# thomasahle/tinyknn

Hardware: AMD Instinct MI355X
Metric: queries/sec at Recall10@10 on GloVe-100 angular (synthetic stand-in), IVF+4-bit PQ, build_probes=1 (higher is better)
Workload: dtype int8 (saturating PQ sums) + f32 (tables, rescoring); 1 GPU; glove-100-angular stand-in: 300 Gaussian clusters sigma 0.7, N=1183514 d=100 IVF n_clusters=1087 build_probes=1 FastPQ dpb=2 M=52; k=10, n_probes=10, parallelism=replica x1 (queries sharded), batches_in_flight=2

## Files before the change

tinyknn_amd/csrc/heap.hip:

```cpp
#include <stdlib.h>

#include <type_traits>

#include "kernels.h"

typedef __attribute__((address_space(3))) volatile uint32_t lds_vu32;
typedef __attribute__((address_space(3))) volatile int32_t lds_vi32;
typedef __attribute__((address_space(3))) volatile int64_t lds_vi64;
#define LDS_PTR(T, p) ((T *)(__attribute__((address_space(3))) unsigned char *)(p))

template <bool SIGNED>
__device__ __forceinline__ bool byte_lt(uint32_t d, uint32_t bound8)
{
    if (SIGNED) return (int)(int8_t)d < (int)(int8_t)bound8;
    return d < bound8;
}

template <bool SIGNED>
__device__ __forceinline__ bool any_lt16(const uint4 v, uint32_t bound8)
{
    const uint32_t w[4] = {v.x, v.y, v.z, v.w};
    bool any = false;
#pragma unroll
    for (int i = 0; i < 4; i++)
// ... 266 lines not shown
#pragma unroll
        for (int i = 0; i < 4; i++) {
            const uint4 dd = dd4[i];
            uint64_t mask = __builtin_amdgcn_ballot_w64(byte_lt<SIGNED>(mn4[i], bound));
            while (mask) {
                const int j = __builtin_ctzll(mask);
                mask &= mask - 1;
                const uint32_t d0 = __builtin_amdgcn_readlane(dd.x, j);
                const uint32_t d1 = __builtin_amdgcn_readlane(dd.y, j);
                const uint32_t d2 = __builtin_amdgcn_readlane(dd.z, j);
                const uint32_t d3 = __builtin_amdgcn_readlane(dd.w, j);
                const int64_t pos0 = 16 * (int64_t)__builtin_amdgcn_readlane(bm4[i], j);
                const uint32_t wr = lane < 4 ? d0 : lane < 8 ? d1 : lane < 12 ? d2 : d3;
                const uint32_t myb = (wr >> (8 * (lane & 3))) & 0xffu;
                uint32_t bits = (uint32_t)__builtin_amdgcn_ballot_w64(lane < 16 && byte_lt<SIGNED>(myb, bound));
                while (bits) {
                    const int r = __builtin_ctz(bits);
                    bits &= bits - 1;
                    const int64_t pos = pos0 + r;
                    if (pos < n) {
                        const uint32_t w = r < 4 ? d0 : r < 8 ? d1 : r < 12 ? d2 : d3;
                        const uint32_t by = (w >> (8 * (r & 3))) & 0xffu;
                        reg_heap_insert(H, K, pos, SIGNED ? (int32_t)(int8_t)by : (int32_t)by);
                    }
                }
                bound = (uint32_t)__builtin_amdgcn_readlane(H.v, 0) & 0xffu;
                if (mask) mask &= __builtin_amdgcn_ballot_w64(byte_lt<SIGNED>(mn4[i], bound));
            }
        }
    }
}

template <bool SIGNED>
__global__ __launch_bounds__(1024) void flat_top_one_kernel(const uint4 *__restrict__ dist,
                                                            const uint8_t *__restrict__ mins, int chunks, int h,
                                                            int64_t n, int R, uint4 *__restrict__ cdist,
                                                            int *__restrict__ cblock, int64_t *__restrict__ out_idx,
                                                            int32_t *__restrict__ out_val)
{
#ifdef TK_FLAT_CLOCK
    int64_t *dbg = (int64_t *)(out_idx + 1024);
    int n_ins = 0;
#define CLK(i) if (tid == 0) { dbg[2 * (i)] = __builtin_readcyclecounter(); dbg[2 * (i) + 1] = __builtin_amdgcn_s_memrealtime(); }
#else
#define CLK(i)
#endif
    __shared__ uint32_t s_bound;
    __shared__ int s_wave[16], s_total;
    const int tid = threadIdx.x, lane = tid & 63, wave = tid >> 6;
    RegHeap H = {SIGNED ? 127 : 255, 0xffffffffu, 0xffffffffu};
    uint32_t bound = SIGNED ? 127u : 255u;
    const RegHeapLane K = reg_heap_lane(lane, R);
    const int rest = chunks - h;
    const int per = ((rest + 1023) / 1024 + 15) & ~15;
    const int b_lo = h + tid * per;
    uint4 pm[4];
#pragma unroll
    for (int g = 0; g < 4; g++) {
        const int b0 = b_lo + 16 * g;
        pm[g] = make_uint4(0, 0, 0, 0);
        if (16 * g < per && b0 < chunks) pm[g] = *(const uint4 *)(mins + b0);
    }
    CLK(0)
    if (wave == 0) {
        reg_heap_span<SIGNED>(H, K, bound, dist, mins, h, nullptr, n, lane);
        if (lane == 0) s_bound = bound;
    }
    CLK(1)
    __syncthreads();
    const uint32_t hb = s_bound;
    uint8_t *cmin = (uint8_t *)(cblock + chunks);
    uint64_t keep = 0;
#pragma unroll
    for (int g = 0; g < 4; g++) {
        const uint32_t w[4] = {pm[g].x, pm[g].y, pm[g].z, pm[g].w};
#pragma unroll
        for (int k = 0; k < 16; k++)
            keep |= (uint64_t)byte_lt<SIGNED>((w[k >> 2] >> (8 * (k & 3))) & 0xffu, hb) << (16 * g + k);
    }
    {
        int valid = per < 64 ? per : 64;
        if (b_lo + valid > chunks) valid = chunks - b_lo;
        keep = valid <= 0 ? 0 : valid >= 64 ? keep : keep & ((1ull << valid) - 1ull);
    }
    int cnt = __builtin_popcountll(keep);
    for (int g = 64; g < per; g += 16) {
        const int b0 = b_lo + g;
        if (b0 >= chunks) break;
        const uint4 m16 = *(const uint4 *)(mins + b0);
        const uint32_t w[4] = {m16.x, m16.y, m16.z, m16.w};
#pragma unroll
        for (int k = 0; k < 16; k++)
            cnt += (b0 + k < chunks) && byte_lt<SIGNED>((w[k >> 2] >> (8 * (k & 3))) & 0xffu, hb);
    }
    int inc = cnt;
#pragma unroll
    for (int o = 1; o < 64; o <<= 1) {
        const int up = __shfl_up(inc, o, 64);
        if (lane >= o) inc += up;
    }
    if (lane == 63) s_wave[wave] = inc;
    __syncthreads();
    int at = inc - cnt;
    for (int w = 0; w < wave; w++) at += s_wave[w];
    if (tid == 1023) s_total = at + cnt;
    while (keep) {
        const int b = b_lo + __builtin_ctzll(keep);
        keep &= keep - 1;
        cdist[at] = dist[b];
        cblock[at] = b;
        cmin[at] = mins[b];
        at++;
    }
    for (int g = 64; g < per; g += 16) {
        const int b0 = b_lo + g;
        if (b0 >= chunks) break;
        const uint4 m16 = *(const uint4 *)(mins + b0);
        const uint32_t w[4] = {m16.x, m16.y, m16.z, m16.w};
#pragma unroll
        for (int k = 0; k < 16; k++)
            if ((b0 + k < chunks) && byte_lt<SIGNED>((w[k >> 2] >> (8 * (k & 3))) & 0xffu, hb)) {
                cdist[at] = dist[b0 + k];
                cblock[at] = b0 + k;
                cmin[at] = (uint8_t)((w[k >> 2] >> (8 * (k & 3))) & 0xffu);
                at++;
            }
    }
    __threadfence();
    __syncthreads();
    if (wave != 0) return;
    CLK(2)
    reg_heap_span<SIGNED>(H, K, bound, cdist, cmin, s_total, cblock, n, lane);
    CLK(3)
#ifdef TK_FLAT_CLOCK
    if (tid == 0) dbg[8] = s_total;
#endif
    if (lane < R) {
        out_idx[lane] = (int64_t)(((uint64_t)H.hi << 32) | H.lo);
        out_val[lane] = H.v;
    }
}

void tk_launch_flat_top_one(const uint4 *dist, const uint8_t *mins, int chunks, int h, int64_t n, int R, int signd,
                            uint4 *cdist, int *cblock, int64_t *out_idx, int32_t *out_val, hipStream_t s)
{
    if (signd)
        hipLaunchKernelGGL(flat_top_one_kernel<true>, dim3(1), dim3(1024), 0, s, dist, mins, chunks, h, n, R, cdist,
                           cblock, out_idx, out_val);
    else
        hipLaunchKernelGGL(flat_top_one_kernel<false>, dim3(1), dim3(1024), 0, s, dist, mins, chunks, h, n, R, cdist,
                           cblock, out_idx, out_val);
}

#ifndef TK_LANES_SEG
#define TK_LANES_SEG 8
#endif
template <bool SIGNED>
__device__ __forceinline__ int entry_val(uint32_t e)
{
    return SIGNED ? ((int32_t)e >> 24) : (int)(e >> 24);
}

template <bool SIGNED>
__device__ __forceinline__ uint32_t mask_lt16(const uint4 v, uint32_t bound8)
{
    const uint32_t w[4] = {v.x, v.y, v.z, v.w};
    uint32_t m = 0;
#pragma unroll
    for (int i = 0; i < 4; i++)
#pragma unroll
        for (int b = 0; b < 4; b++)
            m |= (uint32_t)byte_lt<SIGNED>((w[i] >> (8 * b)) & 0xffu, bound8) << (4 * i + b);
    return m;
}

template <bool SIGNED>
__device__ __forceinline__ uint32_t bound_bytes(uint32_t bound8)
{
    const uint32_t b = SIGNED ? (bound8 ^ 0x80u) : bound8;
    return __builtin_amdgcn_perm(b, b, 0u);
}

template <bool SIGNED>
__device__ __forceinline__ uint32_t lt4(uint32_t x, uint32_t bb, uint32_t bl)
{
    const uint32_t H = 0x80808080u;
    const uint32_t xu = SIGNED ? (x ^ H) : x;
    const uint32_t t = (xu | H) - bl;
    return ((~xu & bb) | (~(xu ^ bb) & ~t)) & H;
}

template <bool SIGNED>
__device__ __forceinline__ uint32_t mask_lt16_swar(const uint4 v, uint32_t bb)
{
    const uint32_t bl = bb & 0x7f7f7f7fu;
    uint32_t lo = __builtin_amdgcn_udot4(lt4<SIGNED>(v.x, bb, bl), 0x08040201u, 0u, false);
    lo = __builtin_amdgcn_udot4(lt4<SIGNED>(v.y, bb, bl), 0x80402010u, lo, false);
    uint32_t hi = __builtin_amdgcn_udot4(lt4<SIGNED>(v.z, bb, bl), 0x08040201u, 0u, false);
    hi = __builtin_amdgcn_udot4(lt4<SIGNED>(v.w, bb, bl), 0x80402010u, hi, false);
    return (lo >> 7) | (hi << 1);
}

template <bool SIGNED>
__global__ void pad_fix_kernel(uint4 *__restrict__ dist, int64_t cap, int64_t nq,
                               const int *__restrict__ slot_prefix, const int *__restrict__ slot_n,
                               int S, int slots_uniform, uint8_t *__restrict__ mins, int64_t cap_min,
                               int *__restrict__ flag_list)
{
    const int64_t i = (int64_t)blockIdx.x * blockDim.x + threadIdx.x;
    if (i == 0 && flag_list) flag_list[0] = 0;
    if (i >= nq * S) return;
    const int64_t q = i / S;
    const int sl = (int)(i - q * S);
    const int64_t qs = slots_uniform ? 0 : q;
    const int f0 = slot_prefix[qs * (S + 1) + sl], f1 = slot_prefix[qs * (S + 1) + sl + 1];
    int n = slot_n[qs * S + sl];
    n = n < 0 ? 0 : n;
    const uint32_t fill = SIGNED ? 0x7f7f7f7fu : 0xffffffffu;
    for (int c = n >> 4; c < f1 - f0; c++) {
        const int keep = n - 16 * c;
        uint4 v = dist[q * cap + f0 + c];
        uint32_t w[4] = {v.x, v.y, v.z, v.w};
        int m = SIGNED ? 127 : 255;
#pragma unroll
        for (int j = 0; j < 4; j++) {
            int km = keep - 4 * j;
            km = km < 0 ? 0 : (km > 4 ? 4 : km);
            const uint32_t kmask = km >= 4 ? 0xffffffffu : ((1u << (8 * km)) - 1u);
            w[j] = (w[j] & kmask) | (fill & ~kmask);
#pragma unroll
            for (int t = 0; t < 4; t++) {
                const uint32_t b = (w[j] >> (8 * t)) & 0xffu;
                const int x = SIGNED ? (int)(int8_t)b : (int)b;
                m = x < m ? x : m;
            }
        }
        dist[q * cap + f0 + c] = make_uint4(w[0], w[1], w[2], w[3]);
        mins[q * cap_min + f0 + c] = (uint8_t)m;
    }
}

template <bool SIGNED, bool DEDUPE, int LW, bool LAZY = false, bool TWIN = false>
__global__ __launch_bounds__(256) void heap_replay_lanes_kernel(
    const uint4 *__restrict__ dist, int64_t cap, int64_t nq, const int *__restrict__ slot_prefix,
    const int *__restrict__ slot_n, const int64_t *__restrict__ slot_label_off, int S,
    const int64_t *__restrict__ labels, int64_t *__restrict__ heap_idx,
    int32_t *__restrict__ heap_val, int R, int slots_uniform,
    unsigned char *__restrict__ skip, int nbuf, const uint8_t *__restrict__ mins,
    int64_t cap_min, const int32_t *__restrict__ labels32, unsigned long long *__restrict__ dbg,
    int prio, int wave_lds, const int *__restrict__ plain0_arr, const int *__restrict__ qlim, const TkTwins tw,
    int *__restrict__ flag_list)
{
    static_assert(!(TWIN && DEDUPE), "one form of the duplicate test");
    if ((prio & 0xff) >= 3) __builtin_amdgcn_s_setprio(3);
    else if ((prio & 0xff) == 2) __builtin_amdgcn_s_setprio(2);
    else if ((prio & 0xff) == 1) __builtin_amdgcn_s_setprio(1);
    extern __shared__ __attribute__((aligned(16))) unsigned char smem_wg[];
    unsigned char *smem = smem_wg + (size_t)(threadIdx.x >> 6) * wave_lds;
    uint32_t *H = (uint32_t *)smem;
    const int R4 = (R + 3) >> 2;
    constexpr size_t CB = (size_t)LW * 4;
    uint32_t *LAB = (uint32_t *)(smem + (size_t)(R + 2) * CB);
    uint4 *TB = (uint4 *)(smem + (size_t)(R + 2) * CB + (size_t)R4 * CB * 4);
    uint4 *ST = (uint4 *)(smem + (size_t)(R + 2) * CB +
                          (DEDUPE ? (size_t)R4 * CB * 4 + (size_t)64 * CB * 4 : 0));
    int *SE = (int *)(ST + (DEDUPE ? 16 : LAZY ? 0 : TWIN ? 16 : TK_LANES_SEG) * LW);
    int *SB = SE + (size_t)S * LW;
    uint4 *PL = (uint4 *)(SB + (size_t)S * LW);
    const int S4 = (S + 3) >> 2;
    uint32_t *BM = (uint32_t *)(PL + (size_t)S4 * LW);
    const int BMW = TWIN ? tw.bm_words : 0;
#define TK_LAB(slot) LAB[(((slot) >> 2) * LW + lane) * 4 + ((slot) & 3)]
    const int lane = threadIdx.x & 63;
    const int64_t q = ((int64_t)blockIdx.x * (blockDim.x >> 6) + (threadIdx.x >> 6)) * LW + lane;
    if (LW < 64 && lane >= LW) return;
    const bool valid = q < nq && !(skip && skip[q]);
    const int64_t qc = q < nq ? q : nq - 1;
    const int64_t qs = slots_uniform ? 0 : qc;
    const int *prefix = slot_prefix + qs * (S + 1);
    const uint4 *drow = dist + qc * cap;

    const uint32_t fresh_val = SIGNED ? 0x7f000000u : 0xff000000u;
    const uint32_t fresh = fresh_val | 0x00ffffffu;
    const uint32_t lowest = SIGNED ? 0x80000000u : 0u;
    for (int j = 0; j < R; j++)
        H[j * LW + lane] = DEDUPE ? (fresh_val | (uint32_t)j) : fresh;
    if (DEDUPE) {
        for (int g = 0; g < R4; g++)
            ((uint4 *)LAB)[g * LW + lane] = make_uint4(~0u, ~0u, ~0u, ~0u);
        for (int b = 0; b < 64; b++) TB[b * LW + lane] = make_uint4(~0u, ~0u, ~0u, ~0u);
    }
    uint32_t sh0 = ~0u, sh1 = ~0u, sh2 = ~0u, sh3 = ~0u;
    bool tb_ovf = false;
    H[R * LW + lane] = H[(R + 1) * LW + lane] = lowest;
#define TK_FRESH(j) (R > (j) ? (DEDUPE ? (fresh_val | (uint32_t)(j)) : fresh) : lowest)
    uint32_t h0 = TK_FRESH(0), h1 = TK_FRESH(1), h2 = TK_FRESH(2), h3 = TK_FRESH(3),
             h4 = TK_FRESH(4), h5 = TK_FRESH(5), h6 = TK_FRESH(6);
#undef TK_FRESH
    uint32_t bound = SIGNED ? 0x7fu : 0xffu;
    uint32_t bb = bound_bytes<SIGNED>(bound);

    const int total = (valid && S > 0) ? prefix[S] : 0;
    const int plain0 = (plain0_arr && valid) ? plain0_arr[qc] : 0x7fffffff;
    uint32_t b_plain = SIGNED ? 0x7fu : 0xffu;
    const uint4 *mrow = (const uint4 *)(mins + qc * cap_min);
    constexpr int SEG = (LAZY || DEDUPE || TWIN) ? 16 : TK_LANES_SEG;
    int nseg = (total + SEG - 1) / SEG;
    int max_nseg = nseg;
    for (int o = LW / 2; o > 0; o >>= 1) {
        int other = __shfl_xor(max_nseg, o, 64);
        max_nseg = other > max_nseg ? other : max_nseg;
    }
    max_nseg = __builtin_amdgcn_readfirstlane(max_nseg);

    int s = 0;
    if (DEDUPE || TWIN) {
        for (int t = 0; t < S; t++) {
            const int e0 = prefix[t], e1 = prefix[t + 1];
            SE[t * LW + lane] = valid ? e1 : 0x7fffffff;
            SB[t * LW + lane] = (int)(slot_label_off[qs * S + t] - 16 * (int64_t)e0);
        }
    }
    int f = 0x7fffffff;
    uint64_t pm = 0;
    int se_cur = 0x7fffffff, sb_cur = 0;
    if (TWIN && S > 0) {
        se_cur = valid ? prefix[1] : 0x7fffffff;
        sb_cur = (int)(slot_label_off[qs * S] - 16 * (int64_t)prefix[0]);
    }
    if (TWIN) {
        const int64_t *pq = tw.probes + qc * S;
        for (int g = 0; g < S4; g++) {
            uint4 pl;
            pl.x = (uint32_t)(int)pq[4 * g];
            pl.y = 4 * g + 1 < S ? (uint32_t)(int)pq[4 * g + 1] : 0x7fffffffu;
            pl.z = 4 * g + 2 < S ? (uint32_t)(int)pq[4 * g + 2] : 0x7fffffffu;
            pl.w = 4 * g + 3 < S ? (uint32_t)(int)pq[4 * g + 3] : 0x7fffffffu;
            PL[g * LW + lane] = pl;
        }
        for (int g = 0; g < BMW; g++) BM[g * LW + lane] = 0;
    }

    const int last_blk = (int)(cap > 0 ? cap - 1 : 0);
    const int last_m = (int)(cap_min / 16) - 1;
    uint4 nx[SEG];
    uint4 mins_nx = make_uint4(0, 0, 0, 0);
#define TK_MINS_ROW16(g_) mrow[(g_) < last_m ? (g_) : (last_m > 0 ? last_m : 0)]
#define TK_MINS_ROW(g_) TK_MINS_ROW16(SEG == 16 ? (g_) : (g_) >> 1)
#define TK_FETCH_BLOCKS(g_)                                                       \
    {                                                                             \
        _Pragma("unroll") for (int k = 0; k < SEG; k++) {                         \
            int blk_ = SEG * (g_) + k;                                            \
            blk_ = blk_ < last_blk ? blk_ : last_blk;                             \
            nx[k] = drow[blk_];                                                   \
        }                                                                         \
    }
#pragma unroll
    for (int k = 0; k < SEG; k++) nx[k] = make_uint4(0, 0, 0, 0);
    uint4 mins_n2 = make_uint4(0, 0, 0, 0), pre = make_uint4(0, 0, 0, 0), pre_n = make_uint4(0, 0, 0, 0);
    int pre_blk = -1, pre_n_blk = -1;
    if (max_nseg > 0) {
        mins_nx = TK_MINS_ROW(0);
        if (LAZY && max_nseg > 1) mins_n2 = TK_MINS_ROW(1);
        if (!LAZY) TK_FETCH_BLOCKS(0)
    }
    int rounds = 0;
    for (int g = 0; g < max_nseg; g++) {
        if (!LAZY) {
#pragma unroll
            for (int k = 0; k < SEG; k++) ST[k * LW + lane] = nx[k];
        }
        const uint4 mins_cur = mins_nx;
        if (LAZY) {
            mins_nx = mins_n2;
            if (g + 2 < max_nseg) mins_n2 = TK_MINS_ROW(g + 2);
            pre = pre_n;
            pre_blk = pre_n_blk;
            pre_n_blk = -1;
            if (g + 1 < max_nseg) {
                int kn = total - 16 * (g + 1);
                kn = kn < 0 ? 0 : (kn > 16 ? 16 : kn);
                uint32_t hn = mask_lt16_swar<SIGNED>(mins_nx, bb);
                hn &= kn >= 16 ? 0xffffu : ((1u << kn) - 1u);
                if (hn) {
                    pre_n_blk = 16 * (g + 1) + __builtin_ctz(hn);
                    pre_n = drow[pre_n_blk < last_blk ? pre_n_blk : last_blk];
                }
            }
        } else if (g + 1 < max_nseg) {
            mins_nx = TK_MINS_ROW(g + 1);
            TK_FETCH_BLOCKS(g + 1)
        }
        const int buf = 0;
        int kmax = total - SEG * g;
        kmax = kmax < 0 ? 0 : (kmax > SEG ? SEG : kmax);
        uint32_t hit = mask_lt16_swar<SIGNED>(mins_cur, bb);
        if (SEG == 8) hit = (hit >> (8 * (g & 1))) & 0xffu;
        hit &= kmax >= SEG ? ((1u << SEG) - 1u) : ((1u << kmax) - 1u);
        uint32_t bits = 0;
        uint4 dd = make_uint4(0, 0, 0, 0);
        int cur = 0;
        uint32_t lab_next = 0;
        int lab_base = 0;
        int tw_next = -1;
#define TK_ADVANCE() \
            while (bits == 0 && hit) { \
                const int k = __builtin_ctz(hit); \
                hit &= hit - 1; \
                cur = SEG * g + k; \
                if (LAZY) { \
                    if (cur == pre_blk) dd = pre; \
                    else dd = drow[cur < last_blk ? cur : last_blk]; \
                } else { \
                    dd = ST[(buf * 16 + k) * LW + lane]; \
                } \
                bits = mask_lt16_swar<SIGNED>(dd, bb); \
                if (DEDUPE && bits) { \
                    while (cur >= SE[s * LW + lane]) s++; \
                    lab_base = SB[s * LW + lane] + 16 * cur; \
                    lab_next = (uint32_t)labels32[(int64_t)lab_base + __builtin_ctz(bits)]; \
                } \
                if (TWIN && bits) { \
                    while (cur >= se_cur) { \
                        const int cs = ((const int *)PL)[(((s >> 2) * LW + lane) << 2) + (s & 3)]; \
                        if (BMW) BM[(cs >> 5) * LW + lane] |= 1u << (cs & 31); \
                        else pm |= 1ull << (cs & 63); \
                        s++; \
                        se_cur = SE[s * LW + lane]; \
                        sb_cur = SB[s * LW + lane]; \
                    } \
                    lab_base = sb_cur + 16 * cur; \
                    if (s > 0) tw_next = tw.list[(lab_base + __builtin_ctz(bits)) * tw.w]; \
                } \
            }
        constexpr bool EARLY = TWIN && !LAZY;
        auto lds_levels = [&](int j, const uint32_t entry, const int v) {
            bool first = true, go = true;
            do {
                const int l = 2 * j + 1;
                const int lc = l < R ? l : R;
                const uint32_t el = H[lc * LW + lane];
                const uint32_t er = H[(lc + 1) * LW + lane];
                const int vl = entry_val<SIGNED>(el), vr = entry_val<SIGNED>(er);
                const bool cl = vl > v;
                const int nvv = cl ? vl : v;
                uint32_t ne = cl ? el : entry;
                int nxt = cl ? l : j;
                const bool cr = vr > nvv;
                ne = cr ? er : ne;
                nxt = cr ? l + 1 : nxt;
                if (first) {
                    h3 = j == 3 ? ne : h3; h4 = j == 4 ? ne : h4;
                    h5 = j == 5 ? ne : h5; h6 = j == 6 ? ne : h6;
                    first = false;
                } else {
                    H[j * LW + lane] = ne;
                }
                go = nxt != j;
                j = nxt;
            } while (go);
        };
        for (;;) {
            if (!EARLY) {
                TK_ADVANCE()
                if (__builtin_amdgcn_ballot_w64(bits != 0) == 0) break;
                rounds++;
            }
            int j = 0;
            uint32_t entry = 0;
            int v = 0;
            if (bits) {
                const int r = __builtin_ctz(bits);
                bits &= bits - 1;
                const uint32_t w = r < 4 ? dd.x : r < 8 ? dd.y : r < 12 ? dd.z : dd.w;
                const uint32_t by = (w >> (8 * (r & 3))) & 0xffu;
                uint32_t low = (uint32_t)(16 * cur + r);
                bool dup = false;
                if (DEDUPE) {
                    const uint32_t label = lab_next;
                    if (bits) lab_next = (uint32_t)labels32[(int64_t)lab_base + __builtin_ctz(bits)];
                    const TkBucketPair lb = tk_label_bucket_pair(label);
                    const int b1 = lb.b1, b2 = lb.b2;
                    const uint4 x1 = TB[b1 * LW + lane], x2 = TB[b2 * LW + lane];
                    dup = (x1.x == label) | (x1.y == label) | (x1.z == label) | (x1.w == label) |
                          (x2.x == label) | (x2.y == label) | (x2.z == label) | (x2.w == label) |
                          (sh0 == label) | (sh1 == label) | (sh2 == label) | (sh3 == label);
                    if (tb_ovf) {
#pragma unroll 4
                        for (int g = 0; g < R4; g++) {
                            const uint4 lv = ((const uint4 *)LAB)[g * LW + lane];
                            dup |= (lv.x == label) | (lv.y == label) | (lv.z == label) | (lv.w == label);
                        }
                    }
                    low = h0 & 0x00ffffffu;
                    const uint32_t gone = TK_LAB(low);
                    if (!dup) {
                        if (gone != 0xffffffffu) {
                            const TkBucketPair gb = tk_label_bucket_pair(gone);
                            const int g1 = gb.b1, g2 = gb.b2;
                            const uint4 y1 = TB[g1 * LW + lane], y2 = TB[g2 * LW + lane];
                            const int p1 = y1.x == gone ? 0 : y1.y == gone ? 1 : y1.z == gone ? 2 : y1.w == gone ? 3 : -1;
                            const int p2 = y2.x == gone ? 0 : y2.y == gone ? 1 : y2.z == gone ? 2 : y2.w == gone ? 3 : -1;
                            if (p1 >= 0) ((uint32_t *)TB)[(g1 * LW + lane) * 4 + p1] = 0xffffffffu;
                            else if (p2 >= 0) ((uint32_t *)TB)[(g2 * LW + lane) * 4 + p2] = 0xffffffffu;
                            else {
                                sh0 = sh0 == gone ? ~0u : sh0; sh1 = sh1 == gone ? ~0u : sh1;
                                sh2 = sh2 == gone ? ~0u : sh2; sh3 = sh3 == gone ? ~0u : sh3;
                            }
                        }
                        const int e1 = (x1.x == ~0u) + (x1.y == ~0u) + (x1.z == ~0u) + (x1.w == ~0u);
                        const int e2 = (x2.x == ~0u) + (x2.y == ~0u) + (x2.z == ~0u) + (x2.w == ~0u);
                        const bool first = e1 >= e2;
                        const uint4 xs = first ? x1 : x2;
                        const int pe = xs.x == ~0u ? 0 : xs.y == ~0u ? 1 : xs.z == ~0u ? 2 : xs.w == ~0u ? 3 : -1;
                        if (pe >= 0) ((uint32_t *)TB)[((first ? b1 : b2) * LW + lane) * 4 + pe] = label;
                        else if (sh0 == ~0u) sh0 = label;
                        else if (sh1 == ~0u) sh1 = label;
                        else if (sh2 == ~0u) sh2 = label;
                        else if (sh3 == ~0u) sh3 = label;
                        else tb_ovf = true;
                        TK_LAB(low) = label;
                    }
                }
                entry = (by << 24) | low;
                v = entry_val<SIGNED>(entry);
                if (TWIN && s > 0) {
                    const int row = lab_base + r;
                    int c = tw_next;
                    if (bits) tw_next = tw.list[(lab_base + __builtin_ctz(bits)) * tw.w];
#pragma nounroll
                    for (int u = 0; u < tw.w && !dup; u++) {
                        if (u > 0) c = tw.list[row * tw.w + u];
                        if (c < 0) break;
                        if (BMW) {
                            if (!((BM[(c >> 5) * LW + lane] >> (c & 31)) & 1u)) continue;
                        } else if (!((pm >> (c & 63)) & 1ull)) continue;
                        if (BMW && v < f) { dup = true; break; }
                        int t = -1;
#pragma nounroll
                        for (int g = 0; g < S4; g++) {
                            const uint4 pl = PL[g * LW + lane];
                            t = ((int)pl.x == c && 4 * g < s) ? 4 * g : t;
                            t = ((int)pl.y == c && 4 * g + 1 < s) ? 4 * g + 1 : t;
                            t = ((int)pl.z == c && 4 * g + 2 < s) ? 4 * g + 2 : t;
                            t = ((int)pl.w == c && 4 * g + 3 < s) ? 4 * g + 3 : t;
                        }
                        if (t < 0) continue;
                        if (v < f) { dup = true; break; }
                        const uint32_t E = (by << 24) | (uint32_t)(16 * prefix[t] + tw.off[row * tw.w + u]);
                        if (v > f) {
                            dup = h0 == E;
                        } else {
                            bool found = (h0 == E) | (h1 == E) | (h2 == E) | (h3 == E) | (h4 == E) | (h5 == E) | (h6 == E);
#pragma nounroll
                            for (int jj = 7; jj < R; jj++) found |= H[jj * LW + lane] == E;
                            dup = found;
                        }
                    }
                }
                if (TWIN && !dup) {
                    const int root = entry_val<SIGNED>(h0);
                    f = root < f ? root : f;
                }
                if (!dup)
                {
                    const int v1 = entry_val<SIGNED>(h1), v2 = entry_val<SIGNED>(h2);
                    const bool c1 = v1 > v;
                    const int nv = c1 ? v1 : v;
                    const bool c2 = v2 > nv;
                    h0 = c2 ? h2 : (c1 ? h1 : entry);
                    if (c1 | c2) {
                        const uint32_t a = c2 ? h5 : h3, b = c2 ? h6 : h4;
                        const int va = entry_val<SIGNED>(a), vb = entry_val<SIGNED>(b);
                        const bool ca = va > v;
                        const int nv1 = ca ? va : v;
                        const bool cb = vb > nv1;
                        const uint32_t ne1 = cb ? b : (ca ? a : entry);
                        if (c2) h2 = ne1; else h1 = ne1;
                        if (ca | cb) {
                            j = (c2 ? 5 : 3) + (cb ? 1 : 0);
                            if (!EARLY) lds_levels(j, entry, v);
                        }
                    }
                }
                if (bits == 0) {
                    bound = h0 >> 24;
                    bb = bound_bytes<SIGNED>(bound);
                    b_plain = cur < plain0 ? bound : b_plain;
                }
            }
            if (EARLY) {
                TK_ADVANCE()
                if (j) lds_levels(j, entry, v);
                if (__builtin_amdgcn_ballot_w64(bits != 0) == 0) break;
                rounds++;
            }
        }
    }
#undef TK_ADVANCE
#undef TK_FETCH_BLOCKS
#undef TK_MINS_ROW
#undef TK_MINS_ROW16
    if (dbg && lane == 0) {
        atomicAdd(&dbg[0], (unsigned long long)rounds);
        atomicMax(&dbg[1], (unsigned long long)rounds);
        atomicAdd(&dbg[2], 1ull);
        atomicAdd(&dbg[3], (unsigned long long)max_nseg);
    }
    if (R > 0) H[0 * LW + lane] = h0;
    if (R > 1) H[1 * LW + lane] = h1;
    if (R > 2) H[2 * LW + lane] = h2;
    if (R > 3) H[3 * LW + lane] = h3;
    if (R > 4) H[4 * LW + lane] = h4;
    if (R > 5) H[5 * LW + lane] = h5;
    if (R > 6) H[6 * LW + lane] = h6;
    if (!valid) {
        if (flag_list && q < nq) flag_list[1 + atomicAdd(&flag_list[0], 1)] = (int)q;
        return;
    }
    if (plain0_arr && plain0 < total && (int)(int8_t)b_plain > qlim[qc]) {
        skip[q] = DEDUPE ? 1 : 2;
        if (flag_list) flag_list[1 + atomicAdd(&flag_list[0], 1)] = (int)q;
    }
    const int64_t *loffs = slot_label_off + qs * S;
    for (int j = 0; j < R; j++) {
        const uint32_t e = H[j * LW + lane];
        const uint32_t pos = e & 0x00ffffffu;
        int64_t label = -1;
        if (DEDUPE) {
            label = (int64_t)(int32_t)TK_LAB(pos);
        } else if (pos != 0x00ffffffu) {
            const int f = (int)(pos >> 4);
            int lo = 0, hi = S;
            while (hi - lo > 1) {
                int mid = (lo + hi) >> 1;
                if (prefix[mid] <= f) lo = mid; else hi = mid;
            }
            const int64_t inlist = (int64_t)pos - 16 * (int64_t)prefix[lo];
            const int64_t loff = loffs[lo];
            label = loff < 0 ? inlist : labels[loff + inlist];
        }
        heap_idx[q * R + j] = label;
        heap_val[q * R + j] = entry_val<SIGNED>(e);
    }
}

template <bool SIGNED, bool DEDUPE>
__global__ __launch_bounds__(64 * TK_HEAP_WAVES) void heap_replay_packed_kernel(
    const uint4 *__restrict__ dist, int64_t cap, const int *__restrict__ slot_prefix,
    const int *__restrict__ slot_n, const int64_t *__restrict__ slot_label_off, int S,
    const int64_t *__restrict__ labels, int64_t *__restrict__ heap_idx,
    int32_t *__restrict__ heap_val, int R, int slots_uniform,
    const unsigned char *__restrict__ flags, int run_if, int64_t nq, const int *__restrict__ flag_list,
    volatile int *host_count)
{
    if (host_count && flag_list && blockIdx.x == 0 && threadIdx.x == 0) *host_count = flag_list[0];
    extern __shared__ __attribute__((aligned(16))) unsigned char smem[];
    const int wave = threadIdx.x >> 6;
    const size_t wstride = DEDUPE ? (((size_t)R * 12 + 15) & ~(size_t)15) : (size_t)R * 4;
    lds_vi64 *lab = LDS_PTR(lds_vi64, smem + wave * wstride);
    lds_vu32 *H = LDS_PTR(lds_vu32, smem + wave * wstride + (DEDUPE ? (size_t)R * 8 : 0));
    const int lane = threadIdx.x & 63;
    const int64_t q = (int64_t)blockIdx.x * (blockDim.x >> 6) + wave;
    if (q >= nq) return;
    if (flags && (run_if < 0 ? flags[q] == 0 : (int)flags[q] != run_if)) return;
    const int64_t qs = slots_uniform ? 0 : q;
    const int *prefix = slot_prefix + qs * (S + 1);
    const uint4 *drow = dist + q * cap;

    const uint32_t fresh_val = SIGNED ? 0x7f000000u : 0xff000000u;
    for (int t = lane; t < R; t += 64) {
        H[t] = fresh_val | (DEDUPE ? (uint32_t)t : 0x00ffffffu);
        if (DEDUPE) lab[t] = -1;
    }
    uint32_t bound = SIGNED ? 0x7fu : 0xffu;
    const uint4 never = SIGNED ? make_uint4(0x7f7f7f7fu, 0x7f7f7f7fu, 0x7f7f7f7fu, 0x7f7f7f7fu)
                               : make_uint4(0xffffffffu, 0xffffffffu, 0xffffffffu, 0xffffffffu);
    for (int s = 0; s < S; s++) {
        const int c0 = prefix[s];
        const int nchunks = prefix[s + 1] - c0;
        const int n = slot_n[qs * S + s];
        const int64_t loff = slot_label_off[qs * S + s];
        const int64_t *labp = loff < 0 ? nullptr : labels + loff;
        for (int base = 0; base < nchunks; base += 64) {
            const int b = base + lane;
            const bool have = b < nchunks;
            uint4 dd = never;
            if (have) dd = drow[c0 + b];
            bool vote = have && any_lt16<SIGNED>(dd, bound);
            uint64_t mask = __builtin_amdgcn_ballot_w64(vote);
            auto load_labels = [&](int jb) -> int64_t {
                const int64_t inl = 16 * (int64_t)(base + jb) + lane;
                if (lane >= 16 || inl >= n) return -2;
                return labp ? labp[inl] : inl;
            };
            int j_pref = -1;
            int64_t lab_pref = -2;
            if (DEDUPE && mask) {
                j_pref = __builtin_ctzll(mask);
                lab_pref = load_labels(j_pref);
            }
            while (mask) {
                const int j = __builtin_ctzll(mask);
                mask &= mask - 1;
                int64_t lab_cur = -2;
                if (DEDUPE) {
                    lab_cur = (j == j_pref) ? lab_pref : load_labels(j);
                    if (mask) {
                        j_pref = __builtin_ctzll(mask);
                        lab_pref = load_labels(j_pref);
                    }
                }
                const uint32_t d0 = __builtin_amdgcn_readlane(dd.x, j);
                const uint32_t d1 = __builtin_amdgcn_readlane(dd.y, j);
                const uint32_t d2 = __builtin_amdgcn_readlane(dd.z, j);
                const uint32_t d3 = __builtin_amdgcn_readlane(dd.w, j);
                const uint32_t w = lane < 4 ? d0 : lane < 8 ? d1 : lane < 12 ? d2 : d3;
                const uint32_t by = (w >> (8 * (lane & 3))) & 0xffu;
                const int rows = n - 16 * (base + j);
                const bool lt = lane < 16 && lane < rows && byte_lt<SIGNED>(by, bound);
                uint32_t bits = (uint32_t)__builtin_amdgcn_ballot_w64(lt);
                if (!bits) continue;
                const uint32_t pos0 = (uint32_t)(16 * (c0 + base + j));
                while (bits) {
                    const int r = __builtin_ctz(bits);
                    bits &= bits - 1;
                    const uint32_t byr = __builtin_amdgcn_readlane(by, r);
                    uint32_t low = pos0 + (uint32_t)r;
                    if (DEDUPE) {
                        const uint32_t llo = __builtin_amdgcn_readlane((uint32_t)lab_cur, r);
                        const uint32_t lhi = __builtin_amdgcn_readlane((uint32_t)((uint64_t)lab_cur >> 32), r);
                        const int64_t label = (int64_t)(((uint64_t)lhi << 32) | llo);
                        bool dup = false;
                        for (int t = lane; t < R; t += 64) dup |= (lab[t] == label);
                        if (__builtin_amdgcn_ballot_w64(dup)) continue;
                        low = __builtin_amdgcn_readfirstlane(H[0]) & 0x00ffffffu;
                        if (lane == 0) lab[low] = label;
                    }
                    const uint32_t entry = (byr << 24) | low;
                    const int v = entry_val<SIGNED>(entry);
                    int jn = 0;
                    for (;;) {
                        const int l = 2 * jn + 1;
                        if (l >= R) { if (lane == 0) H[jn] = entry; break; }
                        uint32_t el = H[l];
                        uint32_t er = (l + 1 < R) ? H[l + 1] : 0u;
                        el = __builtin_amdgcn_readfirstlane(el);
                        er = __builtin_amdgcn_readfirstlane(er);
                        int nxt = jn, nv = v;
                        uint32_t ne = entry;
                        if (entry_val<SIGNED>(el) > nv) { nxt = l; nv = entry_val<SIGNED>(el); ne = el; }
                        if (l + 1 < R && entry_val<SIGNED>(er) > nv) { nxt = l + 1; ne = er; }
                        if (nxt == jn) { if (lane == 0) H[jn] = entry; break; }
                        if (lane == 0) H[jn] = ne;
                        jn = nxt;
                    }
                }
                bound = __builtin_amdgcn_readfirstlane(H[0]) >> 24;
                if (mask) {
                    vote = vote && any_lt16<SIGNED>(dd, bound);
                    mask &= __builtin_amdgcn_ballot_w64(vote);
                }
            }
        }
    }
    const int64_t *loffs = slot_label_off + qs * S;
    for (int t = lane; t < R; t += 64) {
        const uint32_t e = H[t];
        const uint32_t pos = e & 0x00ffffffu;
        int64_t label = -1;
        if (DEDUPE) {
            label = lab[pos];
        } else if (pos != 0x00ffffffu) {
            const int f = (int)(pos >> 4);
            int lo = 0, hi = S;
            while (hi - lo > 1) {
                int mid = (lo + hi) >> 1;
                if (prefix[mid] <= f) lo = mid; else hi = mid;
            }
            const int64_t inlist = (int64_t)pos - 16 * (int64_t)prefix[lo];
            const int64_t loff = loffs[lo];
            label = loff < 0 ? inlist : labels[loff + inlist];
        }
        heap_idx[q * R + t] = label;
        heap_val[q * R + t] = entry_val<SIGNED>(e);
    }
}

void tk_launch_heap_replay_packed(const TkReplayJob &j, const unsigned char *flags, int run_if, bool dedupe,
                                  hipStream_t s, const int *flag_list, int *host_count)
{
    if (j.nq == 0 || j.R == 0) return;
    const size_t wstride = dedupe ? (((size_t)j.R * 12 + 15) & ~(size_t)15) : (size_t)j.R * 4;
    int waves = (int)(64 * 1024 / wstride);
    waves = waves < 1 ? 1 : (waves > TK_HEAP_WAVES ? TK_HEAP_WAVES : waves);
    size_t lds = wstride * waves;
    dim3 grid((unsigned)((j.nq + waves - 1) / waves)), block(64 * waves);
#define TK_LAUNCH(S_, D_)                                                                              \
    hipLaunchKernelGGL((heap_replay_packed_kernel<S_, D_>), grid, block, lds, s, j.dist, j.cap,        \
                       j.slot_prefix, j.slot_n, j.slot_label_off, j.S, j.labels, j.heap_idx, j.heap_val, \
                       j.R, j.slots_uniform, flags, run_if, j.nq, flag_list, host_count)
    if (j.signd) { if (dedupe) TK_LAUNCH(true, true); else TK_LAUNCH(true, false); }
    else { if (dedupe) TK_LAUNCH(false, true); else TK_LAUNCH(false, false); }
#undef TK_LAUNCH
}

#undef TK_LAB

static size_t tk_lanes_fixed_lds(int R, int S, int dedupe)
{
    return (size_t)(R + 2) * 256 + (dedupe ? (size_t)((R + 3) / 4) * 1024 + 65536 + (size_t)S * 512 : 0);
}
static size_t tk_lanes_twin_lds(int R, int S, int bm_words)
{
    return (size_t)(R + 2) * 256 + (size_t)S * 512 + (size_t)((S + 3) / 4) * 1024 + (size_t)bm_words * 256;
}
int tk_lanes_twin_bm_words(int64_t n_lists) { return n_lists <= 4096 ? (int)((n_lists + 31) / 32) : 0; }
int tk_lanes_twin_fits(int R, int S, int64_t n_lists)
{
    return R <= TK_LANES_MAX_R && tk_lanes_twin_lds(R, S, tk_lanes_twin_bm_words(n_lists)) + 16384 <= 160 * 1024;
}

int tk_lanes_dedupe_fits(int R, int S)
{
    return R <= TK_LANES_MAX_R_DEDUPE && tk_lanes_fixed_lds(R, S, 1) + 16384 <= 160 * 1024;
}

int tk_launch_heap_replay_lanes(const TkReplayJob &j, const TkLanesOpts &o, hipStream_t s)
{
    const int64_t nq = j.nq;
    const int R = j.R, S = j.S;
    if (nq == 0 || R == 0) return 0;
    TkPlainCheck c = o.check;
    if (!c.plain0 || !c.qlim || !o.skip || !j.signd) c.plain0 = c.qlim = nullptr;
    const int dedupe = o.labels32 != nullptr;
    const TkTwins *t = o.twins;
    const TkTwins tw = !dedupe && t && t->w > 0 && t->list && t->off && t->probes && !j.slots_uniform ? *t : TkTwins();
    const bool twin = tw.w > 0;
    const int LWr = dedupe ? 32 : 64;
    const size_t st_rows = dedupe ? (size_t)16384 : o.lazy ? 0 : twin ? (size_t)16384 : (size_t)1024 * TK_LANES_SEG;
    const size_t lds = twin ? tk_lanes_twin_lds(R, S, tw.bm_words) + st_rows
                            : tk_lanes_fixed_lds(R, S, dedupe) * LWr / 64 + st_rows * LWr / 64;
    static bool attr_set = false;
    if (!attr_set) {
        const void *fns[] = {(const void *)heap_replay_lanes_kernel<true, false, 64>,
                             (const void *)heap_replay_lanes_kernel<false, false, 64>,
                             (const void *)heap_replay_lanes_kernel<true, true, 32>,
                             (const void *)heap_replay_lanes_kernel<false, true, 32>,
                             (const void *)heap_replay_lanes_kernel<true, false, 64, true>,
                             (const void *)heap_replay_lanes_kernel<false, false, 64, true>,
                             (const void *)heap_replay_lanes_kernel<true, false, 64, false, true>,
                             (const void *)heap_replay_lanes_kernel<false, false, 64, false, true>,
                             (const void *)heap_replay_lanes_kernel<true, false, 64, true, true>,
                             (const void *)heap_replay_lanes_kernel<false, false, 64, true, true>};
        for (const void *f : fns)
            if (hipFuncSetAttribute(f, hipFuncAttributeMaxDynamicSharedMemorySize, 160 * 1024) !=
                hipSuccess)
                return -1;
        attr_set = true;
    }
    {
        const int64_t items = nq * S;
        const unsigned pg = (unsigned)((items + 255) / 256);
        if (items > 0 && j.signd)
            hipLaunchKernelGGL(pad_fix_kernel<true>, dim3(pg), dim3(256), 0, s, (uint4 *)j.dist, j.cap, nq,
                               j.slot_prefix, j.slot_n, S, j.slots_uniform, (uint8_t *)j.mins, j.cap_min, c.flag_list);
        else if (items > 0)
            hipLaunchKernelGGL(pad_fix_kernel<false>, dim3(pg), dim3(256), 0, s, (uint4 *)j.dist, j.cap, nq,
                               j.slot_prefix, j.slot_n, S, j.slots_uniform, (uint8_t *)j.mins, j.cap_min, c.flag_list);
    }
    const int wave_lds = (int)lds;
    const int64_t n_waves = (nq + LWr - 1) / LWr;
    dim3 grid((unsigned)n_waves);
    const int prio = 3;
#define TK_LAUNCH(...)                                                                                          \
    hipLaunchKernelGGL((heap_replay_lanes_kernel<__VA_ARGS__>), grid, dim3(64), lds, s, j.dist, j.cap, nq,            \
                       j.slot_prefix, j.slot_n, j.slot_label_off, S, j.labels, j.heap_idx, j.heap_val, R,             \
                       j.slots_uniform, o.skip, 1, j.mins, j.cap_min, o.labels32, o.counters, prio, wave_lds, \
                       c.plain0, c.qlim, tw, c.flag_list)
    if (dedupe) { if (j.signd) TK_LAUNCH(true, true, 32); else TK_LAUNCH(false, true, 32); }
    else if (twin) {
        if (j.signd) { if (o.lazy) TK_LAUNCH(true, false, 64, true, true); else TK_LAUNCH(true, false, 64, false, true); }
        else { if (o.lazy) TK_LAUNCH(false, false, 64, true, true); else TK_LAUNCH(false, false, 64, false, true); }
    } else if (o.lazy) { if (j.signd) TK_LAUNCH(true, false, 64, true); else TK_LAUNCH(false, false, 64, true); }
    else { if (j.signd) TK_LAUNCH(true, false, 64); else TK_LAUNCH(false, false, 64); }
#undef TK_LAUNCH
    return 0;
}

#define TK_PAIR_LOW (-(1 << 20))

struct PairLane {
    uint32_t anc_mask, anc_bits;
};
__device__ __forceinline__ PairLane pair_lane(int lane)
{
    PairLane K;
    K.anc_mask = K.anc_bits = 0;
    for (int t = lane; t > 0;) {
        const int par = (t - 1) >> 1;
        K.anc_mask |= 1u << par;
        K.anc_bits |= (uint32_t)((t - 1) & 1) << par;
        t = par;
    }
    return K;
}

template <bool SIGNED>
struct PairHeapPos {
    uint32_t e0, e1, er;
    bool right, onp;
    uint32_t ce, fe, ce0;
    int cev, fev;
    __device__ __forceinline__ void init(int lane, int R)
    {
        const uint32_t fresh = SIGNED ? 0x7fffffffu : 0xffffffffu;
        const uint32_t lowest = SIGNED ? 0x80ffffffu : 0x00ffffffu;
        er = fresh;
        e0 = 2 * lane + 1 < R ? fresh : lowest;
        e1 = 2 * lane + 2 < R ? fresh : lowest;
    }
    __device__ __forceinline__ void prepare(int lane, const PairLane &K)
    {
        const uint32_t lowest = SIGNED ? 0x80ffffffu : 0x00ffffffu;
        const int v0 = entry_val<SIGNED>(e0), v1 = entry_val<SIGNED>(e1);
        right = v1 > v0;
        const uint32_t ball = (uint32_t)__builtin_amdgcn_ballot_w64(right);
        onp = ((ball ^ K.anc_bits) & K.anc_mask) == 0;
        ce = right ? e1 : e0;
        cev = right ? v1 : v0;
        const int c = 2 * lane + 1 + (int)right;
        const uint32_t got = (uint32_t)__builtin_amdgcn_ds_bpermute((c & 63) << 2, (int)ce);
        fe = c < 64 ? got : lowest;
        fev = entry_val<SIGNED>(fe);
        ce0 = __builtin_amdgcn_readlane(ce, 0);
    }
    __device__ __forceinline__ uint32_t bound() const { return er >> 24; }
    __device__ __forceinline__ bool holds24(uint32_t l24) const
    {
        const bool here = (((e0 ^ l24) & 0x00ffffffu) == 0) | (((e1 ^ l24) & 0x00ffffffu) == 0);
        return __builtin_amdgcn_ballot_w64(here) != 0 || ((er ^ l24) & 0x00ffffffu) == 0;
    }
    __device__ __forceinline__ void insert(uint32_t e, int v, int lane, const PairLane &K)
    {
        const bool upd = onp && cev > v;
        const uint32_t ne = fev > v ? fe : e;
        e0 = (upd && !right) ? ne : e0;
        e1 = (upd && right) ? ne : e1;
        er = entry_val<SIGNED>(ce0) > v ? ce0 : e;
        prepare(lane, K);
    }
};

template <bool SIGNED>
struct PairHeapLab {
    int v0, v1, vr;
    uint32_t lo0, lo1, lor, hi0, hi1, hir;
    bool right, onp;
    int cev, fev, cev0;
    uint32_t clo, chi, flo, fhi, clo0, chi0;
    __device__ __forceinline__ void init(int lane, int R)
    {
        const int fresh = SIGNED ? 127 : 255;
        vr = fresh;
        v0 = 2 * lane + 1 < R ? fresh : TK_PAIR_LOW;
        v1 = 2 * lane + 2 < R ? fresh : TK_PAIR_LOW;
        lo0 = lo1 = lor = hi0 = hi1 = hir = 0xffffffffu;
    }
    __device__ __forceinline__ void prepare(int lane, const PairLane &K)
    {
        right = v1 > v0;
        const uint32_t ball = (uint32_t)__builtin_amdgcn_ballot_w64(right);
        onp = ((ball ^ K.anc_bits) & K.anc_mask) == 0;
        cev = right ? v1 : v0;
        clo = right ? lo1 : lo0;
        chi = right ? hi1 : hi0;
        const int c = 2 * lane + 1 + (int)right;
        const int a = (c & 63) << 2;
        const int gv = __builtin_amdgcn_ds_bpermute(a, cev);
        const uint32_t gl = (uint32_t)__builtin_amdgcn_ds_bpermute(a, (int)clo);
        const uint32_t gh = (uint32_t)__builtin_amdgcn_ds_bpermute(a, (int)chi);
        fev = c < 64 ? gv : TK_PAIR_LOW;
        flo = gl;
        fhi = gh;
        cev0 = __builtin_amdgcn_readlane(cev, 0);
        clo0 = __builtin_amdgcn_readlane(clo, 0);
        chi0 = __builtin_amdgcn_readlane(chi, 0);
    }
    __device__ __forceinline__ uint32_t bound() const { return (uint32_t)vr & 0xffu; }
    __device__ __forceinline__ bool holds(uint32_t llo, uint32_t lhi) const
    {
        const bool here = ((lo0 == llo) & (hi0 == lhi)) | ((lo1 == llo) & (hi1 == lhi));
        return __builtin_amdgcn_ballot_w64(here) != 0 || (lor == llo && hir == lhi);
// ... 458 lines not shown
```

Before: 26.09 million queries/s.

## Replace segmented block fetch with ring-buffered sparse block prefetch in heap replay

For the plain path (not lazy, dedupe or twin), the kernel no longer loads every block of a fixed segment. It now scans the per-window mins masks and issues loads only for blocks whose minimum beats the current bound. Those loads go into an 8-slot LDS ring, with block deltas packed into 64-bit queues, and the heap updates are interleaved with refills for a bounded number of rounds. The aim is to cut wasted global loads for blocks that cannot enter the top-R and to overlap fetch latency with heap work. In exchange the control flow is more complex and can diverge, and more state is held in registers. The register-level heap update is also factored into a shared lambda.

```diff
diff --git a/tinyknn_amd/csrc/heap.hip b/tinyknn_amd/csrc/heap.hip
--- a/tinyknn_amd/csrc/heap.hip
+++ b/tinyknn_amd/csrc/heap.hip
@@ -442,8 +442,12 @@
                            cblock, out_idx, out_val);
 }
 
-#ifndef TK_LANES_SEG
-#define TK_LANES_SEG 8
+#define TK_RING_SLOTS 8
+#ifndef TK_RING_T
+#define TK_RING_T 4
+#endif
+#ifndef TK_RING_LOADS
+#define TK_RING_LOADS 4
 #endif
 template <bool SIGNED>
 __device__ __forceinline__ int entry_val(uint32_t e)
@@ -554,7 +558,7 @@
     uint4 *TB = (uint4 *)(smem + (size_t)(R + 2) * CB + (size_t)R4 * CB * 4);
     uint4 *ST = (uint4 *)(smem + (size_t)(R + 2) * CB +
                           (DEDUPE ? (size_t)R4 * CB * 4 + (size_t)64 * CB * 4 : 0));
-    int *SE = (int *)(ST + (DEDUPE ? 16 : LAZY ? 0 : TWIN ? 16 : TK_LANES_SEG) * LW);
+    int *SE = (int *)(ST + (DEDUPE ? 16 : LAZY ? 0 : TWIN ? 16 : TK_RING_SLOTS) * LW);
     int *SB = SE + (size_t)S * LW;
     uint4 *PL = (uint4 *)(SB + (size_t)S * LW);
     const int S4 = (S + 3) >> 2;
@@ -594,8 +598,9 @@
     const int plain0 = (plain0_arr && valid) ? plain0_arr[qc] : 0x7fffffff;
     uint32_t b_plain = SIGNED ? 0x7fu : 0xffu;
     const uint4 *mrow = (const uint4 *)(mins + qc * cap_min);
-    constexpr int SEG = (LAZY || DEDUPE || TWIN) ? 16 : TK_LANES_SEG;
-    int nseg = (total + SEG - 1) / SEG;
+    constexpr bool RING = !LAZY && !DEDUPE && !TWIN;
+    constexpr int SEG = 16;
+    int nseg = RING ? 0 : (total + SEG - 1) / SEG;
     int max_nseg = nseg;
     for (int o = LW / 2; o > 0; o >>= 1) {
         int other = __shfl_xor(max_nseg, o, 64);
@@ -636,7 +641,7 @@
     uint4 nx[SEG];
     uint4 mins_nx = make_uint4(0, 0, 0, 0);
 #define TK_MINS_ROW16(g_) mrow[(g_) < last_m ? (g_) : (last_m > 0 ? last_m : 0)]
-#define TK_MINS_ROW(g_) TK_MINS_ROW16(SEG == 16 ? (g_) : (g_) >> 1)
+#define TK_MINS_ROW(g_) TK_MINS_ROW16(g_)
 #define TK_FETCH_BLOCKS(g_)                                                       \
     {                                                                             \
         _Pragma("unroll") for (int k = 0; k < SEG; k++) {                         \
@@ -649,13 +654,143 @@
     for (int k = 0; k < SEG; k++) nx[k] = make_uint4(0, 0, 0, 0);
     uint4 mins_n2 = make_uint4(0, 0, 0, 0), pre = make_uint4(0, 0, 0, 0), pre_n = make_uint4(0, 0, 0, 0);
     int pre_blk = -1, pre_n_blk = -1;
-    if (max_nseg > 0) {
+    if (!RING && max_nseg > 0) {
         mins_nx = TK_MINS_ROW(0);
         if (LAZY && max_nseg > 1) mins_n2 = TK_MINS_ROW(1);
         if (!LAZY) TK_FETCH_BLOCKS(0)
     }
     int rounds = 0;
-    for (int g = 0; g < max_nseg; g++) {
+    auto lds_levels = [&](int j, const uint32_t entry, const int v) {
+        bool first = true, go = true;
+        do {
+            const int l = 2 * j + 1;
+            const int lc = l < R ? l : R;
+            const uint32_t el = H[lc * LW + lane];
+            const uint32_t er = H[(lc + 1) * LW + lane];
+            const int vl = entry_val<SIGNED>(el), vr = entry_val<SIGNED>(er);
+            const bool cl = vl > v;
+            const int nvv = cl ? vl : v;
+            uint32_t ne = cl ? el : entry;
+            int nxt = cl ? l : j;
+            const bool cr = vr > nvv;
+            ne = cr ? er : ne;
+            nxt = cr ? l + 1 : nxt;
+            if (first) {
+                h3 = j == 3 ? ne : h3; h4 = j == 4 ? ne : h4;
+                h5 = j == 5 ? ne : h5; h6 = j == 6 ? ne : h6;
+                first = false;
+            } else {
+                H[j * LW + lane] = ne;
+            }
+            go = nxt != j;
+            j = nxt;
+        } while (go);
+    };
+    auto reg_levels = [&](const uint32_t entry, const int v) -> int {
+        const int v1 = entry_val<SIGNED>(h1), v2 = entry_val<SIGNED>(h2);
+        const bool c1 = v1 > v;
+        const int nv = c1 ? v1 : v;
+        const bool c2 = v2 > nv;
+        h0 = c2 ? h2 : (c1 ? h1 : entry);
+        if (!(c1 | c2)) return 0;
+        const uint32_t a = c2 ? h5 : h3, b = c2 ? h6 : h4;
+        const int va = entry_val<SIGNED>(a), vb = entry_val<SIGNED>(b);
+        const bool ca = va > v;
+        const int nv1 = ca ? va : v;
+        const bool cb = vb > nv1;
+        const uint32_t ne1 = cb ? b : (ca ? a : entry);
+        if (c2) h2 = ne1; else h1 = ne1;
+        return (ca | cb) ? (c2 ? 5 : 3) + (cb ? 1 : 0) : 0;
+    };
+    int refills = 0;
+    if constexpr (RING) {
+        const int nwin = (total + 15) >> 4;
+        int win = -1;
+        uint32_t wmask = 0;
+        uint4 m1 = make_uint4(0, 0, 0, 0), m2 = m1;
+        const bool wave_rows = __builtin_amdgcn_ballot_w64(nwin > 0) != 0;
+        if (wave_rows) {
+            m1 = TK_MINS_ROW16(0);
+            m2 = TK_MINS_ROW16(1);
+        }
+        int head = 0, nst = 0, nfl = 0;
+        uint64_t qlo = 0, qhi = 0;
+        int last_req = 0;
+        uint4 fl[TK_RING_LOADS];
+#pragma unroll
+        for (int k = 0; k < TK_RING_LOADS; k++) fl[k] = make_uint4(0, 0, 0, 0);
+        uint32_t bits = 0;
+        uint4 dd = make_uint4(0, 0, 0, 0);
+        int cur = 0;
+        while (wave_rows) {
+            const bool more = nfl > 0 || wmask != 0 || win + 1 < nwin;
+            refills += __builtin_amdgcn_ballot_w64(more) != 0;
+#pragma unroll
+            for (int k = 0; k < TK_RING_LOADS; k++)
+                if (k < nfl) ST[((head + nst + k) & (TK_RING_SLOTS - 1)) * LW + lane] = fl[k];
+            nst += nfl;
+            nfl = 0;
+#pragma unroll
+            for (int a = 0; a < 2; a++) {
+                if (wmask == 0 && win + 1 < nwin) {
+                    win++;
+                    const int kn = total - 16 * win;
+                    wmask = mask_lt16_swar<SIGNED>(a ? m2 : m1, bb) & (kn >= 16 ? 0xffffu : ((1u << kn) - 1u));
+                    if (16 * win - last_req > 0xffe0) wmask |= 1u;
+                }
+            }
+            int room = TK_RING_SLOTS - nst;
+            room = room > TK_RING_LOADS ? TK_RING_LOADS : room;
+#pragma unroll
+            for (int k = 0; k < TK_RING_LOADS; k++) {
+                const bool take = k < room && wmask != 0;
+                const int blk = take ? 16 * win + __builtin_ctz(wmask) : last_req;
+                wmask &= take ? wmask - 1 : ~0u;
+                fl[k] = drow[blk < last_blk ? blk : last_blk];
+                const int p = nst + nfl;
+                const uint64_t step = (uint64_t)(uint32_t)(blk - last_req) << (16 * (p & 3));
+                qlo |= take && p < 4 ? step : 0;
+                qhi |= take && p >= 4 ? step : 0;
+                last_req = blk;
+                nfl += take;
+            }
+            m1 = TK_MINS_ROW16(win + 1);
+            m2 = TK_MINS_ROW16(win + 2);
+            const bool rest = __builtin_amdgcn_ballot_w64(nfl > 0 || wmask != 0 || win + 1 < nwin) != 0;
+            bool any = true;
+            for (int t = 0; rest ? t < TK_RING_T : true; t++) {
+                while (bits == 0 && nst > 0) {
+                    dd = ST[head * LW + lane];
+                    head = (head + 1) & (TK_RING_SLOTS - 1);
+                    nst--;
+                    cur += (int)((uint32_t)qlo & 0xffffu);
+                    qlo = (qlo >> 16) | (qhi << 48);
+                    qhi >>= 16;
+                    bits = mask_lt16_swar<SIGNED>(dd, bb);
+                }
+                any = __builtin_amdgcn_ballot_w64(bits != 0) != 0;
+                if (!any) break;
+                rounds++;
+                if (bits) {
+                    const int r = __builtin_ctz(bits);
+                    bits &= bits - 1;
+                    const uint32_t w = r < 4 ? dd.x : r < 8 ? dd.y : r < 12 ? dd.z : dd.w;
+                    const uint32_t by = (w >> (8 * (r & 3))) & 0xffu;
+                    const uint32_t entry = (by << 24) | (uint32_t)(16 * cur + r);
+                    const int v = entry_val<SIGNED>(entry);
+                    const int j = reg_levels(entry, v);
+                    if (j) lds_levels(j, entry, v);
+                    if (bits == 0) {
+                        bound = h0 >> 24;
+                        bb = bound_bytes<SIGNED>(bound);
+                        b_plain = cur < plain0 ? bound : b_plain;
+                    }
+                }
+            }
+            if (!rest) break;
+        }
+    }
+    for (int g = 0; !RING && g < max_nseg; g++) {
         if (!LAZY) {
 #pragma unroll
             for (int k = 0; k < SEG; k++) ST[k * LW + lane] = nx[k];
@@ -685,7 +820,6 @@
         int kmax = total - SEG * g;
         kmax = kmax < 0 ? 0 : (kmax > SEG ? SEG : kmax);
         uint32_t hit = mask_lt16_swar<SIGNED>(mins_cur, bb);
-        if (SEG == 8) hit = (hit >> (8 * (g & 1))) & 0xffu;
         hit &= kmax >= SEG ? ((1u << SEG) - 1u) : ((1u << kmax) - 1u);
         uint32_t bits = 0;
         uint4 dd = make_uint4(0, 0, 0, 0);
@@ -724,32 +858,6 @@
                 } \
             }
         constexpr bool EARLY = TWIN && !LAZY;
-        auto lds_levels = [&](int j, const uint32_t entry, const int v) {
-            bool first = true, go = true;
-            do {
-                const int l = 2 * j + 1;
-                const int lc = l < R ? l : R;
-                const uint32_t el = H[lc * LW + lane];
-                const uint32_t er = H[(lc + 1) * LW + lane];
-                const int vl = entry_val<SIGNED>(el), vr = entry_val<SIGNED>(er);
-                const bool cl = vl > v;
-                const int nvv = cl ? vl : v;
-                uint32_t ne = cl ? el : entry;
-                int nxt = cl ? l : j;
-                const bool cr = vr > nvv;
-                ne = cr ? er : ne;
-                nxt = cr ? l + 1 : nxt;
-                if (first) {
-                    h3 = j == 3 ? ne : h3; h4 = j == 4 ? ne : h4;
-                    h5 = j == 5 ? ne : h5; h6 = j == 6 ? ne : h6;
-                    first = false;
-                } else {
-                    H[j * LW + lane] = ne;
-                }
-                go = nxt != j;
-                j = nxt;
-            } while (go);
-        };
         for (;;) {
             if (!EARLY) {
                 TK_ADVANCE()
@@ -852,26 +960,9 @@
                     const int root = entry_val<SIGNED>(h0);
                     f = root < f ? root : f;
                 }
-                if (!dup)
-                {
-                    const int v1 = entry_val<SIGNED>(h1), v2 = entry_val<SIGNED>(h2);
-                    const bool c1 = v1 > v;
-                    const int nv = c1 ? v1 : v;
-                    const bool c2 = v2 > nv;
-                    h0 = c2 ? h2 : (c1 ? h1 : entry);
-                    if (c1 | c2) {
-                        const uint32_t a = c2 ? h5 : h3, b = c2 ? h6 : h4;
-                        const int va = entry_val<SIGNED>(a), vb = entry_val<SIGNED>(b);
-                        const bool ca = va > v;
-                        const int nv1 = ca ? va : v;
-                        const bool cb = vb > nv1;
-                        const uint32_t ne1 = cb ? b : (ca ? a : entry);
-                        if (c2) h2 = ne1; else h1 = ne1;
-                        if (ca | cb) {
-                            j = (c2 ? 5 : 3) + (cb ? 1 : 0);
-                            if (!EARLY) lds_levels(j, entry, v);
-                        }
-                    }
+                if (!dup) {
+                    j = reg_levels(entry, v);
+                    if (j && !EARLY) lds_levels(j, entry, v);
                 }
                 if (bits == 0) {
                     bound = h0 >> 24;
@@ -895,7 +986,7 @@
         atomicAdd(&dbg[0], (unsigned long long)rounds);
         atomicMax(&dbg[1], (unsigned long long)rounds);
         atomicAdd(&dbg[2], 1ull);
-        atomicAdd(&dbg[3], (unsigned long long)max_nseg);
+        atomicAdd(&dbg[3], (unsigned long long)(RING ? refills : max_nseg));
     }
     if (R > 0) H[0 * LW + lane] = h0;
     if (R > 1) H[1 * LW + lane] = h1;
@@ -1128,7 +1219,7 @@
     const TkTwins tw = !dedupe && t && t->w > 0 && t->list && t->off && t->probes && !j.slots_uniform ? *t : TkTwins();
     const bool twin = tw.w > 0;
     const int LWr = dedupe ? 32 : 64;
-    const size_t st_rows = dedupe ? (size_t)16384 : o.lazy ? 0 : twin ? (size_t)16384 : (size_t)1024 * TK_LANES_SEG;
+    const size_t st_rows = dedupe ? (size_t)16384 : o.lazy ? 0 : twin ? (size_t)16384 : (size_t)1024 * TK_RING_SLOTS;
     const size_t lds = twin ? tk_lanes_twin_lds(R, S, tw.bm_words) + st_rows
                             : tk_lanes_fixed_lds(R, S, dedupe) * LWr / 64 + st_rows * LWr / 64;
     static bool attr_set = false;
```

Result: faster. 26.99 million queries/s, median of 6 (+3.5%).
